# sacs-epfl/decentralizepy

Hardware: AMD Instinct MI355X
Metric: GiB/s fp32 params encoded+decoded (device-resident), 1% top-k (higher is better)
Workload: dtype f32

## Files before the change

### decentralizepy_amd/csrc/dpz_topk.h

```cpp
#pragma once
#include <cstdlib>

#include "dpz_common.h"
#include "dpz_replace.h"

namespace dpz {

struct KeySrc {
  const float* x;
  const float* x0;
  float* acc;
  int mode;
  int rekey;
};

struct Raw4 {
  float4 a, b, q;
  int cnt;
};

template <bool VEC, bool ACC = true>
__device__ __forceinline__ void load_raw4(const KeySrc& s, int64_t i0, int64_t n, Raw4& r) {
  const int64_t rem = n - i0;
  r.cnt = rem >= 4 ? 4 : (rem > 0 ? (int)rem : 0);
// ... 163 lines not shown
  int64_t R = (n + W - 1) / W;
  R = (R + 31) & ~int64_t(31);
  W = (n + R - 1) / R;
  int64_t cap = ((R / 4) + 63) & ~int64_t(63);
  if (k > n / 16) {
    const double frac = 1.25 * (double)k / (double)n + 0.05;
    cap = ((int64_t)(frac * (double)R) + 63) & ~int64_t(63);
    if (cap > ((R + 63) & ~int64_t(63))) cap = (R + 63) & ~int64_t(63);
  }
  if (cap < 64) cap = 64;
  if (k <= n / 16 && cap > 1024) cap = 1024;
  g.W = W; g.B = (W + 3) / 4; g.R = R; g.CAP = cap;
  return g;
}

static inline size_t align256(size_t v) { return (v + 255) & ~size_t(255); }

struct WsLayout {
  size_t ctrl, chist, ex_hist, ex_gt, ex_eq, ex_off, ex_eqb;
  size_t f_ghist, f_segcnt, f_blkabove, f_blkoff, f_cidx, f_ckey, f_cval, f_blcnt, f_blkey, f_blidx;
  size_t total;
  int64_t ex_nblk;
  FastGeom fg;
};

static inline WsLayout ws_layout(int64_t n, int64_t k = 0, int geom = GEOM_LONE) {
  WsLayout L;
  size_t o = 0;
  L.ex_nblk = (n + EX_CHUNK - 1) / EX_CHUNK;
  if (L.ex_nblk < 1) L.ex_nblk = 1;
  L.fg = fast_geom(n > 0 ? n : 1, k, geom);
  L.ctrl = o; o += align256(sizeof(TopkCtrl));
  L.chist = o; o += align256(CB * 4);
  L.ex_hist = o; o += align256(4096 * 4);
  L.ex_gt = o; o += align256(L.ex_nblk * 4);
  L.ex_eq = o; o += align256(L.ex_nblk * 4);
  L.ex_off = o; o += align256(L.ex_nblk * 4);
  L.ex_eqb = o; o += align256(L.ex_nblk * 4);
  L.f_ghist = o; o += align256(GH_COPIES * GH_STRIDE * 4);
  L.f_blcnt = o; o += align256(NSUB * 4);
  L.f_segcnt = o; o += align256(L.fg.W * 4);
  L.f_blkabove = o; o += align256(L.fg.B * 4);
  L.f_blkoff = o; o += align256(L.fg.B * 4);
  L.f_cidx = o; o += align256((size_t)L.fg.W * L.fg.CAP * 4);
  L.f_ckey = o; o += align256((size_t)L.fg.W * L.fg.CAP * 4);
  L.f_cval = o; o += align256((size_t)L.fg.W * L.fg.CAP * 4);
  L.f_blkey = o; o += align256((size_t)BCAP * 4);
  L.f_blidx = o; o += align256((size_t)BCAP * 4);
  L.total = o;
  return L;
}

static inline size_t ws_bytes_needed(int64_t n, int64_t k) {
  size_t m = 0;
  for (int geom = GEOM_LONE; geom <= GEOM_PIPE; ++geom) {
    const size_t t = ws_layout(n, k, geom).total;
    if (t > m) m = t;
// ... 67 lines not shown
```

### decentralizepy_amd/csrc/dpz_topk_sampled.hip

```cpp
#include <cstdio>
#include <cstdlib>

#include "dpz_topk.h"

namespace dpz {

#ifndef DPZ_FILTER_NT
#define DPZ_FILTER_NT 1
#endif

#ifdef DPZ_STAMPS
__device__ unsigned long long g_stamps[64];
#define STAMP_MIN(i) do { if (threadIdx.x == 0) atomicMin(&g_stamps[i], __builtin_amdgcn_s_memrealtime()); } while (0)
#define STAMP_MAX(i) do { __syncthreads(); if (threadIdx.x == 0) atomicMax(&g_stamps[i], __builtin_amdgcn_s_memrealtime()); } while (0)
#define STAMP_ONE(i) do { if (threadIdx.x == 0) g_stamps[i] = __builtin_amdgcn_s_memrealtime(); } while (0)
__device__ unsigned long long g_bst[16][4096];
#define STAMP_T0(i) do { if (threadIdx.x == 0 && blockIdx.x < 4096) g_bst[i][blockIdx.x] = __builtin_amdgcn_s_memrealtime(); } while (0)
__device__ unsigned long long g_fst[6][8192];
#define STAMP_W(i) do { const int64_t _sg = (int64_t)blockIdx.x * 4 + (threadIdx.x >> 6); if ((threadIdx.x & 63) == 0 && _sg < 8192) g_fst[i][_sg] = __builtin_amdgcn_s_memrealtime(); } while (0)
#else
#define STAMP_T0(i) do {} while (0)
#define STAMP_W(i) do {} while (0)
#define STAMP_MIN(i) do {} while (0)
#define STAMP_MAX(i) do {} while (0)
// ... 516 lines not shown
  const int src = m ? (int)__ffsll((long long)m) - 1 : 0;
  *bstar = __shfl(fb, src, 64);
  *need = __shfl(fn, src, 64);
  return ok;
}

template <int NT>
struct SelectLds {
  uint32_t gh[GH_STRIDE];
  uint32_t lkey[SEL_LCAP], lidx[SEL_LCAP];
  uint32_t fbabove[NT / 64 * 2 / 4];
  uint32_t lcnt, gbase, sb_bstar, sb_need, sb_ok;
};

template <bool VEC, int NT = 1024>
__device__ __forceinline__ void sampled_select_kernel_body(SelectLds<NT>& M, KeySrc s, int64_t n, int64_t k, int64_t W, int64_t B, int64_t R, int64_t CAP, TopkCtrl* ctrl, const uint32_t* __restrict__ ghist, const uint32_t* __restrict__ segcnt, const uint32_t* __restrict__ cidx, const uint32_t* __restrict__ ckey, uint32_t* blkabove, uint32_t* blcnt, uint32_t* blkey, uint32_t* blidx, ReplaceJob pj, const uint32_t BID) {
  static_assert(NT == 1024 || NT == 256, "select block: 1024 or 256 threads");
  constexpr int SS = NT / 64 * 2;
  constexpr int NQ = HB / NT;
  {
    const int64_t own = ((W + SEL_SEGS - 1) / SEL_SEGS) * (SEL_SEGS / SS);
    if ((int64_t)BID >= own) {
      replace_block(pj, (int64_t)BID - own);
      return;
    }
  }
  STAMP_MIN(6);
  STAMP_T0(8);
  uint32_t* const gh = M.gh;
  uint32_t* const fbabove = M.fbabove;
  uint32_t* const lkey = M.lkey;
// ... 131 lines not shown
      const int64_t beg = seg * R;
      const int64_t end = (beg + R < n) ? beg + R : n;
      for (int64_t i0 = beg + lane * 4; i0 - lane * 4 < end; i0 += 256) {
        uint32_t key[4];
        const int c = i0 < end ? load_keys4<VEC>(s, i0, end, false, key) : 0;
#pragma unroll
        for (int e = 0; e < 4; ++e) {
          const bool valid = e < c && key[e] >= lo;
          const uint32_t b = valid ? fine_bin(key[e], lo, hi, shift) : 0u;
          above += (uint32_t)__popcll(__ballot(valid && b > bstar));
          append(valid && b == bstar, key[e], (uint32_t)(i0 + e));
        }
      }
    }
    if (lane == 0 && above) atomicAdd(&fbabove[(wid * 2 + u) >> 2], above);
  }
  __syncthreads();
  if (t < SS / 4) {
    const int64_t fb = (int64_t)BID * (SS / 4) + t;
    blkabove[fb] = fb < B ? fbabove[t] : 0u;
  }
  STAMP_T0(10);
  const uint32_t nl = lcnt;
  if (nl) {
    const int sub = (int)(BID & (NSUB - 1));
    if (t == 0) gbase = atomicAdd(&blcnt[sub], nl > SEL_LCAP ? (uint32_t)BCAP : nl);
    __syncthreads();
    const uint32_t gb = gbase;
    for (uint32_t j = t; j < nl && j < SEL_LCAP; j += NT) {
      const uint32_t p = gb + j;
      if (p < SUBCAP) {
        blkey[sub * SUBCAP + p] = lkey[j];
        blidx[sub * SUBCAP + p] = lidx[j];
      }
    }
  }
  STAMP_T0(11);
}

template <bool VEC>
__global__ void __launch_bounds__(1024) sampled_select_kernel(KeySrc s, int64_t n, int64_t k, int64_t W, int64_t B, int64_t R, int64_t CAP, TopkCtrl* ctrl, const uint32_t* __restrict__ ghist, const uint32_t* __restrict__ segcnt, const uint32_t* __restrict__ cidx, const uint32_t* __restrict__ ckey, uint32_t* blkabove, uint32_t* blcnt, uint32_t* blkey, uint32_t* blidx, ReplaceJob pj) {
  __shared__ __attribute__((aligned(16))) SelectLds<1024> lds;
  sampled_select_kernel_body<VEC>(lds, s, n, k, W, B, R, CAP, ctrl, ghist, segcnt, cidx, ckey, blkabove, blcnt, blkey, blidx, pj, (uint32_t)blockIdx.x);
}

__device__ __forceinline__ uint32_t bound_slot(const uint32_t* subbase, uint32_t j) {
  int sb = 0;
#pragma unroll
  for (int u = 1; u < NSUB; ++u) sb += subbase[u] <= j ? 1 : 0;
  return (uint32_t)sb * SUBCAP + (j - subbase[sb]);
}

constexpr int BLDS = 1024;
struct Bound {
  const uint32_t* key;
  const uint32_t* idx;
  const uint32_t* subbase;
  uint32_t* sk;
// ... 146 lines not shown
}

__device__ __forceinline__ uint64_t block_sum64(uint64_t v, uint64_t* wsum64) {
  const int wid = threadIdx.x >> 6, lane = threadIdx.x & 63;
#pragma unroll
  for (int d = 32; d >= 1; d >>= 1) v += __shfl_xor(v, d, 64);
  if (lane == 0) wsum64[wid] = v;
  __syncthreads();
  uint64_t tot = 0;
  for (int w = 0; w < (int)(blockDim.x >> 6); ++w) tot += wsum64[w];
  __syncthreads();
  return tot;
}

template <bool VEC>
__device__ __forceinline__ uint32_t dense_count(const KeySrc s, int64_t seg, int64_t R,
                                                          int64_t n, uint32_t lo, uint32_t T,
                                                          uint32_t icut) {
  const int lane = threadIdx.x & 63;
  const int64_t beg = seg * R;
  const int64_t end = (beg + R < n) ? beg + R : n;
  uint32_t mine = 0;
  for (int64_t i0 = beg + lane * 4; i0 - lane * 4 < end; i0 += 256) {
    uint32_t key[4];
    const int c = i0 < end ? load_keys4<VEC>(s, i0, end, false, key) : 0;
#pragma unroll
    for (int e = 0; e < 4; ++e) {
      const bool f = e < c && key[e] >= lo &&
                     (key[e] > T || (key[e] == T && (uint32_t)(i0 + e) <= icut));
      mine += (uint32_t)__popcll(__ballot(f));
    }
  }
  return mine;
}

template <bool VEC>
__device__ __forceinline__ void dense_write(const KeySrc s, int64_t seg, int64_t R,
                                                      int64_t n, int64_t k, uint32_t lo,
                                                      uint32_t T, uint32_t icut, uint32_t run,
                                                      const float* vals_src, int32_t* idx_out,
                                                      float* val_out, int32_t* counter,
                                                      float* rewind, int val_h,
                                                      uint32_t* slrow) {
  const int lane = threadIdx.x & 63;
  const int64_t beg = seg * R;
  const int64_t end = (beg + R < n) ? beg + R : n;
  for (int64_t i0 = beg + lane * 4; i0 - lane * 4 < end; i0 += 256) {
    uint32_t key[4];
    const int c = i0 < end ? load_keys4<VEC>(s, i0, end, false, key) : 0;
    bool f[4];
    uint32_t pre = 0, tot = 0;
#pragma unroll
// ... 9 lines not shown
    for (int e = 0; e < 4; ++e) {
      if (f[e]) {
        if (pos < (uint64_t)k) {
          const int64_t i = i0 + e;
          idx_out[pos] = (int32_t)i;
          store_val(val_out, val_h, pos, vals_src[i]);
          if (slrow) atomicOr(&slrow[(i - beg) >> 5], 1u << (i & 31));
          if (counter) atomicAdd(&counter[i], 1);
          if (rewind) rewind[i] = 0.0f;
        }
        ++pos;
      }
    }
    run += tot;
  }
}

template <int SPW>
struct CompactCfg {
  static constexpr int CSEG = 4 * SPW;
  static constexpr int PFC = SPW >= 8 ? 1 : 4;
};

#ifndef DPZ_SL_PF
#define DPZ_SL_PF 4
#endif
constexpr int SL_PF = DPZ_SL_PF;
static_assert(32 % SL_PF == 0, "the planes are read in whole steps");

template <int SPW, bool SL>
struct CompactLds {
  uint32_t slrows[SL ? 4 : 1][SL ? (int)(SL_RMAX / 32) : 1];
  uint32_t wcnt[CompactCfg<SPW>::CSEG];
  uint32_t subbase[NSUB + 1];
  uint32_t flag, spec;
  uint64_t wsum64[4];
  alignas(16) ResolveLds RL;
  alignas(16) uint32_t bsk[BLDS];
  alignas(16) uint32_t bsi[BLDS];
};

template <bool VEC, bool PLAIN, int SPW, bool SL>
__device__ __forceinline__ void sampled_compact_kernel_body(CompactLds<SPW, SL>& M, KeySrc s, int64_t n, int64_t k, int64_t W, int64_t R, int64_t CAP, TopkCtrl* ctrl, uint32_t* chist, const uint32_t* __restrict__ blkabove, const uint32_t* __restrict__ blcnt, const uint32_t* __restrict__ blkey, const uint32_t* __restrict__ blidx, const uint32_t* __restrict__ segcnt, const uint32_t* __restrict__ cidx, const uint32_t* __restrict__ ckey, const float* __restrict__ cval, const float* vals_src, int32_t* idx_out, float* val_out, int32_t* counter, float* rewind, int32_t* status_out, ReplaceJob pj, int64_t nrep_first, int val_h, uint32_t* selmask, uint32_t* planes, int64_t nwords, uint32_t* ghist, uint32_t sig, const uint32_t BID) {
  constexpr int CSEG = CompactCfg<SPW>::CSEG;
  constexpr int PFC = CompactCfg<SPW>::PFC;
  uint32_t* const wcnt = M.wcnt;
  uint32_t* const subbase = M.subbase;
  uint32_t& flag = M.flag;
  uint32_t& spec = M.spec;
  uint64_t* const wsum64 = M.wsum64;
  ResolveLds& RL = M.RL;
  uint32_t* const bsk = M.bsk;
  uint32_t* const bsi = M.bsi;
  const int64_t CB_ = (W + CSEG - 1) / CSEG;
  const int64_t B = (W + 3) / 4;
  if (nrep_first > 0 ? (int64_t)BID < nrep_first : (int64_t)BID >= CB_) {
    replace_block(pj, nrep_first > 0 ? (int64_t)BID : (int64_t)BID - CB_);
    return;
// ... 17 lines not shown
  {
    const uint32_t fb0 = (uint32_t)t * 8u;
    uint4 v0 = make_uint4(0, 0, 0, 0), v1 = make_uint4(0, 0, 0, 0);
    if ((int64_t)fb0 < B) {
      v0 = reinterpret_cast<const uint4*>(blkabove)[2 * t];
      v1 = reinterpret_cast<const uint4*>(blkabove)[2 * t + 1];
    }
    const uint32_t v[8] = {v0.x, v0.y, v0.z, v0.w, v1.x, v1.y, v1.z, v1.w};
    const uint32_t fbx = blk * (uint32_t)(CSEG / 4);
#pragma unroll
    for (int q = 0; q < 8; ++q) {
      abv_all += v[q];
      abv_before += fb0 + q < fbx ? v[q] : 0u;
    }
  }
  uint32_t cnt[SPW], kk[SPW][PFC], ii[SPW][PFC];
  float vv[SPW][PFC];
#pragma unroll
  for (int u = 0; u < SPW; ++u) {
    const int64_t seg = seg0 + u;
    cnt[u] = seg < W ? segcnt[seg] : 0u;
#pragma unroll
    for (int c = 0; c < PFC; ++c) {
      kk[u][c] = 0u;
      ii[u][c] = 0u;
      vv[u][c] = 0.f;
    }
    kk[u][0] = seg < W ? ckey[seg * CAP + lane] : 0u;
    ii[u][0] = seg < W ? cidx[seg * CAP + lane] : 0u;
    if (cval && seg < W) vv[u][0] = cval[seg * CAP + lane];
// ... 15 lines not shown
    for (int c = 0; c < PFC; ++c) cc[u][c] = 0u;
#pragma unroll
  for (int u = 0; u < SPW; ++u) {
    const int64_t seg = seg0 + u;
    if (seg < W && cnt[u] != DENSE && (uint32_t)lane < cnt[u]) {
      if (!cval) vv[u][0] = vals_src[ii[u][0]];
      if (PLAIN && counter) cc[u][0] = (uint32_t)counter[ii[u][0]];
    }
  }
  if (t < 64) {
    uint32_t tot;
    const uint32_t ex = wave_excl_scan(sc, &tot);
    const bool over = __ballot(sc > (uint32_t)SUBCAP) != 0;
    const bool spec_ok = __ballot(sc > SPEC) == 0;
    if (t < NSUB) subbase[t] = ex;
    if (t == 0) {
      subbase[NSUB] = tot;
      flag = (over || tot > (uint32_t)BCAP || need_l == 0 || need_l > tot) ? 1u : 0u;
      spec = spec_ok ? 1u : 0u;
    }
  }
  __syncthreads();
  if (flag) {
    if (blk == 0 && t == 0) {
      ctrl->status = 1;
      atomicOr(&ctrl->sticky, 1u);
      if (status_out) *status_out = 1;
    }
    return;
  }
// ... 8 lines not shown
  if (spec) {
    if (sp_slot < subbase[sp_sub + 1] - subbase[sp_sub]) {
      bsk[subbase[sp_sub] + sp_slot] = spk;
      bsi[subbase[sp_sub] + sp_slot] = spi;
    }
    __syncthreads();
  } else {
    bd.load();
  }
  uint32_t T, icut;
  block_resolve(bd, need, lo + (bstar << shift), shift, RL, &T, &icut);
  T = __builtin_amdgcn_readfirstlane(T);
  icut = __builtin_amdgcn_readfirstlane(icut);
  STAMP_T0(2);
  const uint32_t bstart = (uint32_t)((int64_t)blk * CSEG * R);
  uint32_t sb_before = 0, sb_all = 0;
  bd.each([&](uint32_t kv, uint32_t iv) {
    const bool sel = kv > T || (kv == T && iv <= icut);
    sb_all += sel ? 1u : 0u;
    sb_before += (sel && iv < bstart) ? 1u : 0u;
  });
  const uint64_t tot2 = block_sum64(((uint64_t)(abv_all + sb_all) << 32) |
                                        (uint64_t)(abv_before + sb_before), wsum64);
  const uint32_t boff = __builtin_amdgcn_readfirstlane((uint32_t)tot2);
  const uint32_t grand = __builtin_amdgcn_readfirstlane((uint32_t)(tot2 >> 32));
  if (blk == 0 && t == 0) {
    ctrl->T = T;
    ctrl->icut = icut;
    if (grand != (uint32_t)k) {
      ctrl->status = 2;
      atomicOr(&ctrl->sticky, 2u);
    } else if (T > 0u && T < 0x7F800000u) {
      ctrl->hint_T = T;
      ctrl->hint_sig = sig;
    } else {
// ... 14 lines not shown
            kk[u][c] = ckey[seg * CAP + j];
            ii[u][c] = cidx[seg * CAP + j];
            if (cval) vv[u][c] = cval[seg * CAP + j];
          }
        }
#pragma unroll
        for (int c = 1; c < PFC; ++c) {
          const uint32_t j = c * 64u + lane;
          if (j < cnt[u] && !cval) vv[u][c] = vals_src[ii[u][c]];
          if (PLAIN && counter && j < cnt[u]) cc[u][c] = (uint32_t)counter[ii[u][c]];
        }
      }
    }
  }
  auto is_sel = [&](uint32_t key, uint32_t idx) { return key > T || (key == T && idx <= icut); };
#pragma unroll
  for (int u = 0; u < SPW; ++u) {
    const int64_t seg = seg0 + u;
    uint32_t mine = 0;
    if (seg < W && cnt[u] != DENSE) {
#pragma unroll
      for (int c = 0; c < PFC; ++c) {
        const uint32_t j = c * 64u + lane;
        mine += (uint32_t)__popcll(__ballot(j < cnt[u] && is_sel(kk[u][c], ii[u][c])));
      }
      for (uint32_t j0 = PFC * 64u; j0 < cnt[u]; j0 += 4 * 64u) {
        uint32_t kg[4];
#pragma unroll
        for (int g = 0; g < 4; ++g) {
          const uint32_t j = j0 + g * 64u + lane;
          kg[g] = ckey[seg * CAP + (j < cnt[u] ? j : 0u)];
        }
#pragma unroll
        for (int g = 0; g < 4; ++g) {
          const uint32_t j = j0 + g * 64u + lane;
          bool sel = false;
          if (j < cnt[u]) sel = kg[g] > T || (kg[g] == T && cidx[seg * CAP + j] <= icut);
          mine += (uint32_t)__popcll(__ballot(sel));
        }
      }
    } else if (seg < W) {
      mine = dense_count<VEC>(s, seg, R, n, lo, T, icut);
    }
    if (lane == 0) wcnt[wid * SPW + u] = mine;
  }
  __syncthreads();
  STAMP_T0(3);
  uint32_t run = boff;
  for (int w = 0; w < wid * SPW; ++w) run += wcnt[w];
  run = __builtin_amdgcn_readfirstlane(run);
  uint32_t* const slrow = SL ? M.slrows[wid] : nullptr;
#pragma unroll
  for (int u = 0; u < SPW; ++u) {
    const int64_t seg = seg0 + u;
    if (seg >= W) break;
    const int64_t segbeg = seg * R;
    const int segw = SL ? (int)((((segbeg + R < n) ? segbeg + R : n) - segbeg + 31) >> 5) : 0;
    if (SL) {
      for (int j = lane; j < segw; j += 64) slrow[j] = 0u;
      __builtin_amdgcn_wave_barrier();
    }
// ... 29 lines not shown
          const uint32_t j = j0 + g * 64u + lane;
          const uint32_t jc = seg * CAP + (j < cnt[u] ? j : 0u);
          kg[g] = ckey[jc];
          ig[g] = cidx[jc];
          vg[g] = cval ? cval[jc] : 0.f;
        }
#pragma unroll
        for (int g = 0; g < 4; ++g) {
          const uint32_t j = j0 + g * 64u + lane;
          const bool sel = j < cnt[u] && is_sel(kg[g], ig[g]);
          const uint32_t cw = (PLAIN && counter && sel) ? (uint32_t)counter[ig[g]] : 0u;
          emit(sel, ig[g], vg[g], false, cw);
        }
      }
    } else {
      dense_write<VEC>(s, seg, R, n, k, lo, T, icut, run, vals_src, idx_out, val_out, counter,
                       rewind, val_h, slrow);
      run += wcnt[wid * SPW + u];
    }
    if (SL) {
      __builtin_amdgcn_fence(__ATOMIC_RELEASE, "wavefront");
      __builtin_amdgcn_wave_barrier();
      for (int j = lane; j < segw; j += 64) {
        const uint32_t m = slrow[j];
        const int64_t w = (segbeg >> 5) + j;
        selmask[w] = m;
        uint32_t carry = planes ? m : 0u;
        for (int p = 0; p < 32 && carry != 0u; p += SL_PF) {
          uint32_t o[SL_PF];
#pragma unroll
          for (int q = 0; q < SL_PF; ++q) o[q] = planes[(int64_t)(p + q) * nwords + w];
#pragma unroll
          for (int q = 0; q < SL_PF; ++q) {
            if (carry != 0u) {
              planes[(int64_t)(p + q) * nwords + w] = o[q] ^ carry;
              carry &= o[q];
            }
          }
        }
      }
      __builtin_amdgcn_wave_barrier();
    }
  }
  STAMP_T0(4);
}

template <bool VEC, bool PLAIN, int SPW, bool SL>
__global__ void __launch_bounds__(256, SPW >= 8 ? 1 : 4) sampled_compact_kernel(KeySrc s, int64_t n, int64_t k, int64_t W, int64_t R, int64_t CAP, TopkCtrl* ctrl, uint32_t* chist, const uint32_t* __restrict__ blkabove, const uint32_t* __restrict__ blcnt, const uint32_t* __restrict__ blkey, const uint32_t* __restrict__ blidx, const uint32_t* __restrict__ segcnt, const uint32_t* __restrict__ cidx, const uint32_t* __restrict__ ckey, const float* __restrict__ cval, const float* vals_src, int32_t* idx_out, float* val_out, int32_t* counter, float* rewind, int32_t* status_out, ReplaceJob pj, int64_t nrep_first, int val_h, uint32_t* selmask, uint32_t* planes, int64_t nwords, uint32_t* ghist, uint32_t sig) {
  __shared__ __attribute__((aligned(16))) CompactLds<SPW, SL> lds;
  sampled_compact_kernel_body<VEC, PLAIN, SPW, SL>(lds, s, n, k, W, R, CAP, ctrl, chist, blkabove, blcnt, blkey, blidx, segcnt, cidx, ckey, cval, vals_src, idx_out, val_out, counter, rewind, status_out, pj, nrep_first, val_h, selmask, planes, nwords, ghist, sig, (uint32_t)blockIdx.x);
}

static void cosched_shares(double f[3]) {
  f[0] = 0.45; f[1] = 0.55; f[2] = 0.0;
  if (const char* e = DPZ_KNOB_STR(COSCHED)) {
    double v[3];
    if (sscanf(e, "%lf,%lf,%lf", &v[0], &v[1], &v[2]) == 3 && v[0] >= 0 && v[1] >= 0 &&
        v[2] >= 0) {
      const double t = v[0] + v[1] + v[2];
      if (t > 0)
        for (int i = 0; i < 3; ++i) f[i] = v[i] / t;
    }
  }
}

template <bool VEC>
static int run_sampled_t(const EncodeArgs& a, const WsLayout& L, int phases) {
  KeySrc s{a.x, a.x0, a.acc, a.acc_mode, 0};
  TopkCtrl* ctrl = reinterpret_cast<TopkCtrl*>(a.ws + L.ctrl);
  uint32_t* chist = reinterpret_cast<uint32_t*>(a.ws + L.chist);
  uint32_t* ghist = reinterpret_cast<uint32_t*>(a.ws + L.f_ghist);
  uint32_t* segcnt = reinterpret_cast<uint32_t*>(a.ws + L.f_segcnt);
  uint32_t* blkabove = reinterpret_cast<uint32_t*>(a.ws + L.f_blkabove);
  uint32_t* cidx = reinterpret_cast<uint32_t*>(a.ws + L.f_cidx);
  uint32_t* ckey = reinterpret_cast<uint32_t*>(a.ws + L.f_ckey);
  float* cval = (a.vals_src == a.x) ? reinterpret_cast<float*>(a.ws + L.f_cval) : nullptr;
  uint32_t* blcnt = reinterpret_cast<uint32_t*>(a.ws + L.f_blcnt);
  uint32_t* blkey = reinterpret_cast<uint32_t*>(a.ws + L.f_blkey);
  uint32_t* blidx = reinterpret_cast<uint32_t*>(a.ws + L.f_blidx);
  const FastGeom& g = L.fg;
  const unsigned nb = (unsigned)g.B;
  const unsigned nsel = (unsigned)((g.W + SEL_SEGS - 1) / SEL_SEGS);
  ReplaceJob jb[3] = {};
  unsigned pb[3] = {0, 0, 0};
  const int smp_threads = DPZ_KNOB_INT(SAMPLE_THREADS, 256) == 1024 ? 1024 : 256;
  const int smp_blocks = SMP_NCHUNK / (4 * (smp_threads / 64));
  float* copy_out = (a.job && phases == 3 && a.job->scatter) ? a.job->out : nullptr;
  if (a.job && phases == 3) {
// ... 70 lines not shown
#undef DPZ_PIPE2
#undef DPZ_PIPE1
#undef DPZ_PIPE
    } else if (a.acc_mode == DPZ_ACC_NONE)
      DPZ_TIMED(DPZ_KT_TOPK_FILTER, a.st, sampled_filter_kernel<VEC, false, FG><<<nb, 256, 0, a.st>>>(
          s, a.n, r_lo, r_hi, g.W, g.R, g.CAP, ctrl, chist, ghist, segcnt, cidx, ckey, cval,
          copy_out));
    else
      DPZ_TIMED(DPZ_KT_TOPK_FILTER, a.st, sampled_filter_kernel<VEC, true, 3><<<nb, 256, 0, a.st>>>(
          s, a.n, r_lo, r_hi, g.W, g.R, g.CAP, ctrl, chist, ghist, segcnt, cidx, ckey, cval,
          copy_out));
  }
  if (!(phases & 2)) return DPZ_OK;
  s.rekey = 1;
  DPZ_TIMED(DPZ_KT_TOPK_SELECT, a.st, sampled_select_kernel<VEC><<<nsel + pb[1], 1024, 0, a.st>>>(
      s, a.n, a.k, g.W, g.B, g.R, g.CAP, ctrl, ghist, segcnt, cidx, ckey, blkabove, blcnt, blkey,
      blidx, jb[1]));
  float* rewind = (a.acc && a.acc_mode != DPZ_ACC_NONE && !a.selmask) ? a.acc : nullptr;
  const int ablate = (int)DPZ_KNOB_INT(COMPACT_ABLATE, 0);
  if (ablate & 1) rewind = nullptr;
  int32_t* const counter = ((ablate & 2) || a.selmask) ? nullptr : a.counter;
  const bool plain = DPZ_KNOB_INT(COUNTER_PLAIN, a.k > a.n / 32 ? 1 : 0) != 0;
  const int64_t nrep_first = DPZ_KNOB_INT(SCATTER_FIRST, 0) != 0 ? (int64_t)pb[2] : 0;
  const int spw = (int)DPZ_KNOB_INT(COMPACT_SPW, 2);
#define DPZ_COMPACT(PL_, SPW_, SL_)                                                               \
  DPZ_TIMED(DPZ_KT_TOPK_COMPACT, a.st,                                                            \
            (sampled_compact_kernel<VEC, PL_, SPW_, SL_><<<(unsigned)((g.W + 4 * SPW_ - 1) /       \
                                                                     (4 * SPW_)) + pb[2],         \
                                                           256, 0, a.st>>>(                       \
                s, a.n, a.k, g.W, g.R, g.CAP, ctrl, chist, blkabove, blcnt, blkey, blidx, segcnt, \
                cidx, ckey, cval, a.vals_src, a.idx_out, a.val_out, counter, rewind,              \
                a.status_out, jb[2], nrep_first, a.val_h, a.selmask, a.planes, mask_words(a.n),  \
                ghist, sig)))
  if (a.selmask && g.R <= SL_RMAX) {
    DPZ_COMPACT(false, 2, true);
  } else if (plain) {
    if (spw == 8) DPZ_COMPACT(true, 8, false);
    else DPZ_COMPACT(true, 2, false);
  } else {
    if (spw == 8) DPZ_COMPACT(false, 8, false);
    else DPZ_COMPACT(false, 2, false);
  }
#undef DPZ_COMPACT
  return DPZ_OK;
}

// ... 17 lines not shown
}
#endif

struct EncNode {
  const float* x;
  const float* x0;
  int32_t* counter;
  int32_t* idx_out;
  float* val_out;
  char* ws;
  int32_t* status_out;
  uint64_t pad;
};
static_assert(sizeof(EncNode) == 64, "node table entry: 8 x 64-bit words (dpz_codec.h)");
struct WsOff {
  uint64_t ctrl, chist, ghist, segcnt, blkabove, cidx, ckey, cval, blcnt, blkey, blidx;
};

template <class T>
__host__ __device__ __forceinline__ T* wsp(char* ws, uint64_t off) {
  return reinterpret_cast<T*>(ws + off);
}

__global__ void __launch_bounds__(1024) nodes_sample_kernel(const EncNode* __restrict__ tab,
                                                            WsOff o, int64_t n, int nsb) {
  const uint32_t node = blockIdx.x / (uint32_t)nsb, bid = blockIdx.x % (uint32_t)nsb;
  const EncNode e = tab[node];
  KeySrc s{e.x, e.x0, nullptr, DPZ_ACC_NONE, 0};
  sampled_sample_kernel_body(s, n, wsp<TopkCtrl>(e.ws, o.ctrl), wsp<uint32_t>(e.ws, o.chist),
                             wsp<uint32_t>(e.ws, o.ghist), wsp<uint32_t>(e.ws, o.blcnt),
                             ReplaceJob{}, nsb, 0, bid);
// ... 16 lines not shown
}

__global__ void __launch_bounds__(1024) nodes_select_kernel(const EncNode* __restrict__ tab,
                                                            WsOff o, int64_t n, int64_t k,
                                                            int64_t W, int64_t B, int64_t R,
                                                            int64_t CAP, uint32_t nsel) {
  const uint32_t node = blockIdx.x / nsel, bid = blockIdx.x % nsel;
  const EncNode e = tab[node];
  KeySrc s{e.x, e.x0, nullptr, DPZ_ACC_NONE, 1};
  __shared__ __attribute__((aligned(16))) SelectLds<1024> lds;
  sampled_select_kernel_body<true>(
      lds, s, n, k, W, B, R, CAP, wsp<TopkCtrl>(e.ws, o.ctrl),
      wsp<const uint32_t>(e.ws, o.ghist),
      wsp<const uint32_t>(e.ws, o.segcnt), wsp<const uint32_t>(e.ws, o.cidx),
      wsp<const uint32_t>(e.ws, o.ckey), wsp<uint32_t>(e.ws, o.blkabove),
      wsp<uint32_t>(e.ws, o.blcnt), wsp<uint32_t>(e.ws, o.blkey), wsp<uint32_t>(e.ws, o.blidx),
      ReplaceJob{}, bid);
}

#ifndef DPZ_NODES_NO_COUNTER
#define DPZ_NODES_NO_COUNTER 0
#endif
template <bool PLAIN, bool SL>
__global__ void __launch_bounds__(256, 4) nodes_compact_kernel(const EncNode* __restrict__ tab,
                                                               WsOff o, int64_t n, int64_t k,
                                                               int64_t W, int64_t R, int64_t CAP,
                                                               uint32_t ncb, int64_t nwords,
                                                               uint32_t sig) {
  const uint32_t node = blockIdx.x / ncb, bid = blockIdx.x % ncb;
  const EncNode e = tab[node];
  KeySrc s{e.x, e.x0, nullptr, DPZ_ACC_NONE, 1};
  int32_t* const counter = SL || DPZ_NODES_NO_COUNTER ? nullptr : e.counter;
  uint32_t* const selmask = SL ? reinterpret_cast<uint32_t*>(e.pad) : nullptr;
  uint32_t* const planes = SL ? reinterpret_cast<uint32_t*>(e.counter) : nullptr;
  __shared__ __attribute__((aligned(16))) CompactLds<2, SL> lds;
  sampled_compact_kernel_body<true, PLAIN, 2, SL>(
      lds, s, n, k, W, R, CAP, wsp<TopkCtrl>(e.ws, o.ctrl), wsp<uint32_t>(e.ws, o.chist),
      wsp<const uint32_t>(e.ws, o.blkabove), wsp<const uint32_t>(e.ws, o.blcnt),
      wsp<const uint32_t>(e.ws, o.blkey), wsp<const uint32_t>(e.ws, o.blidx),
      wsp<const uint32_t>(e.ws, o.segcnt), wsp<const uint32_t>(e.ws, o.cidx),
      wsp<const uint32_t>(e.ws, o.ckey), wsp<const float>(e.ws, o.cval), e.x, e.idx_out,
      e.val_out, counter, nullptr, e.status_out, ReplaceJob{}, 0, 0, selmask, planes, nwords,
      wsp<uint32_t>(e.ws, o.ghist), sig, bid);
}

int topk_encode_nodes(int m, const void* table, int64_t n, int64_t k, size_t ws_bytes, int flags,
                      hipStream_t st) {
  if (m < 1 || !table || n <= 0 || n >= (int64_t(1) << 31) || k < 1 || k > n) return DPZ_ERR_ARG;
  if (flags & ~(DPZ_TOPK_HINT | DPZ_TOPK_SLICED)) return DPZ_ERR_ARG;
  if (!use_sampled(n, k)) return DPZ_ERR_UNSUPPORTED;
  const bool sl = (flags & DPZ_TOPK_SLICED) != 0;
  if (ws_bytes < ws_bytes_needed(n, k)) return DPZ_ERR_WORKSPACE;
  const WsLayout L = ws_layout(n, k, true);
  const FastGeom& g = L.fg;
  const WsOff o{L.ctrl, L.chist, L.f_ghist, L.f_segcnt, L.f_blkabove, L.f_cidx, L.f_ckey,
                L.f_cval, L.f_blcnt, L.f_blkey, L.f_blidx};
  const EncNode* tab = static_cast<const EncNode*>(table);
  const uint32_t sig = hint_signature(n, k, true, DPZ_ACC_NONE, true);
  const uint32_t hsig = (flags & DPZ_TOPK_HINT) ? sig : 0u;
  const int nsb = SMP_NCHUNK / 16;
  const uint32_t nb = (uint32_t)g.B, nsel = (uint32_t)((g.W + SEL_SEGS - 1) / SEL_SEGS);
  const uint32_t ncb = (uint32_t)((g.W + 7) / 8);
  if ((uint64_t)m * nb >= (1ull << 31) || (uint64_t)m * ncb >= (1ull << 31)) return DPZ_ERR_ARG;
  if (sl && (g.R > SL_RMAX || (g.R & 31) != 0)) return DPZ_ERR_UNSUPPORTED;
  if (!hsig)
    DPZ_TIMED(DPZ_KT_TOPK_SAMPLE, st,
              nodes_sample_kernel<<<(unsigned)(m * nsb), 256, 0, st>>>(tab, o, n, nsb));
  uint32_t r_lo, r_hi;
  window_ranks(n, k, &r_lo, &r_hi);
  if (g.W > 4096)
// ... 108 lines not shown
  }
  uint32_t bid = blockIdx.x;
  if constexpr (FILTER) {
    if (nf) {
      if (bid < nf) {
        sampled_filter_pipe_kernel_body<1, 1, 4, 4, true>(
            lds.f, fs, n, r_lo, r_hi, W, R, CAP, f_ctrl, f_chist, f_ghist, f_segcnt, f_cidx,
            f_ckey, f_cval, f_out, FoldBase{}, f_hsig, f_blcnt, 0, bid);
        return;
      }
      bid -= nf;
    }
  }
  if (bid < nc) {
    sampled_compact_kernel_body<true, false, 2, false>(
        lds.c, cs, n, k, W, R, CAP, c_ctrl, c_chist, c_blkabove, c_blcnt, c_blkey, c_blidx,
        c_segcnt, c_cidx, c_ckey, c_cval, cs.x, c_idx_out, c_val_out, c_counter, nullptr, nullptr,
        c_pj, 0, 0, nullptr, nullptr, 0, c_ghist, sig, bid);
    return;
  }
  bid -= nc;
  if (bid < nsel) {
    sampled_select_kernel_body<true, 256>(lds.s, ss, n, k, W, B, R, CAP, s_ctrl, s_ghist,
                                          s_segcnt, s_cidx, s_ckey, s_blkabove, s_blcnt, s_blkey,
                                          s_blidx, ReplaceJob{}, bid);
    return;
  }
  bid -= nsel;
  if constexpr (FILTER) {
    if (nf) return;
    sampled_filter_pipe_kernel_body<1, 1, 4, 4, true>(
        lds.f, fs, n, r_lo, r_hi, W, R, CAP, f_ctrl, f_chist, f_ghist, f_segcnt, f_cidx, f_ckey,
        f_cval, f_out, FoldBase{}, f_hsig, f_blcnt, 0, bid);
  }
}

bool topk_pipe_ok(int64_t n, int64_t k, size_t ws_bytes) {
  if (n <= 0 || n >= (int64_t(1) << 31) || !use_sampled(n, k) || k > n / 32) return false;
  if (ws_bytes < ws_bytes_needed(n, k)) return false;
  const int64_t wcap = DPZ_KNOB_INT(WPIPE, 0) > W_PIPE ? (int64_t)W_MAX : (int64_t)W_PIPE;
  return fast_geom(n, k, GEOM_PIPE).W <= wcap && DPZ_KNOB_INT(FILTER_PIPE, 1) > 0;
}

int topk_pipe_chain(int p, const PipeStep* c, int64_t n, int64_t k, int64_t r_k, int mode,
                    hipStream_t st) {
  if (p < 1 || !c || !topk_pipe_ok(n, k, ws_bytes_needed(n, k)) || r_k < 1 || r_k > n)
    return DPZ_ERR_ARG;
  const WsLayout L = ws_layout(n, k, GEOM_PIPE);
  const FastGeom& g = L.fg;
  const WsOff o{L.ctrl, L.chist, L.f_ghist, L.f_segcnt, L.f_blkabove, L.f_cidx, L.f_ckey,
                L.f_cval, L.f_blcnt, L.f_blkey, L.f_blidx};
  const uint32_t sig = hint_signature(n, k, GEOM_PIPE, DPZ_ACC_NONE, true);
  const int nsb = SMP_NCHUNK / 16;
  const uint32_t nb = (uint32_t)g.B;
  const uint32_t nsel1024 = (uint32_t)((g.W + SEL_SEGS - 1) / SEL_SEGS);
  const uint32_t nsel256 = nsel1024 * 4;
  const uint32_t ncb = (uint32_t)((g.W + 7) / 8);
  const uint32_t nsc = (uint32_t)((scatter_chunks(r_k) + 3) / 4);
  uint32_t r_lo, r_hi;
  window_ranks(n, k, &r_lo, &r_hi);
  const bool full = mode >= 2;
  const bool ffirst = DPZ_KNOB_INT(PIPE_ORDER, 1) != 0;
  auto* kmerged = pipe_step_kernel<true, PIPE_OCC>;
  auto* kdrain = pipe_step_kernel<false, PIPE_OCC>;
#ifdef DPZ_DIAG
// ... 55 lines not shown
                    KeySrc{fp.x, fp.x0, nullptr, DPZ_ACC_NONE, 0}, fp.ctrl, fp.chist, fp.ghist,
                    fp.segcnt, fp.cidx, fp.ckey, fp.cval, fp.blcnt, fp.out, fp.hsig,
                    KeySrc{sp.x, sp.x0, nullptr, DPZ_ACC_NONE, 1}, sp.ctrl, sp.ghist, sp.segcnt,
                    sp.cidx, sp.ckey, sp.blkabove, sp.blcnt, sp.blkey, sp.blidx,
                    KeySrc{cp.x, cp.x0, nullptr, DPZ_ACC_NONE, 1}, cp.ctrl, cp.chist, cp.blkabove,
                    cp.blcnt, cp.blkey, cp.blidx, cp.segcnt, cp.cidx, cp.ckey, cp.cval, cp.ghist,
                    cp.idx_out, cp.val_out, cp.counter, cp.pj, n, k, r_lo, r_hi, g.W, g.B, g.R,
                    g.CAP, nc, ns, ffirst ? nf : 0u, sig, poison));
    if (!full && fs) {
      KeySrc s{fs->x, fs->x0, nullptr, DPZ_ACC_NONE, 1};
      DPZ_TIMED(DPZ_KT_TOPK_SELECT, st,
                sampled_select_kernel<true><<<nsel1024, 1024, 0, st>>>(
                    s, n, k, g.W, g.B, g.R, g.CAP, wsp<TopkCtrl>(fs->ws, o.ctrl),
                    wsp<const uint32_t>(fs->ws, o.ghist), wsp<const uint32_t>(fs->ws, o.segcnt),
                    wsp<const uint32_t>(fs->ws, o.cidx), wsp<const uint32_t>(fs->ws, o.ckey),
                    wsp<uint32_t>(fs->ws, o.blkabove), wsp<uint32_t>(fs->ws, o.blcnt),
                    wsp<uint32_t>(fs->ws, o.blkey), wsp<uint32_t>(fs->ws, o.blidx), ReplaceJob{}));
    }
  }
  return DPZ_OK;
}

bool fused_foldbase_ok(const EncodeArgs& a, bool vec) {
  return vec && a.acc_mode == DPZ_ACC_NONE && a.x0 && aligned16(a.base_out) &&
         DPZ_KNOB_INT(FILTER_PIPE, 1) > 0 && use_sampled(a.n, a.k) && !a.job;
}

int run_sampled(const EncodeArgs& a, const WsLayout& L, bool vec, int phases) {
  return vec ? run_sampled_t<true>(a, L, phases) : run_sampled_t<false>(a, L, phases);
}

// ... 2 lines not shown
```

Measured before the change: 1518.

## Reuse per-segment above counts from select to skip compact's counting pass

The select kernel now stores each segment's count of keys strictly above the boundary bin into a new workspace array. The compact kernel seeds its per-wave counts from this array and adds boundary-bin selections with shared-memory atomics. This removes the separate pass that re-read candidates, or the dense segment data, just to count selected elements before writing. The cost is an extra workspace array, a per-segment global store, and a reliance on the segabove offset lining up with the layout in the pipelined path.

```diff
diff --git a/decentralizepy_amd/csrc/dpz_topk.h b/decentralizepy_amd/csrc/dpz_topk.h
--- a/decentralizepy_amd/csrc/dpz_topk.h
+++ b/decentralizepy_amd/csrc/dpz_topk.h
@@ -201,11 +201,15 @@
   return g;
 }
 
-static inline size_t align256(size_t v) { return (v + 255) & ~size_t(255); }
+__host__ __device__ static inline size_t align256(size_t v) { return (v + 255) & ~size_t(255); }
+__host__ __device__ static inline size_t segabove_words(int64_t B) {
+  return align256((size_t)B * 4) / 4;
+}
 
 struct WsLayout {
   size_t ctrl, chist, ex_hist, ex_gt, ex_eq, ex_off, ex_eqb;
-  size_t f_ghist, f_segcnt, f_blkabove, f_blkoff, f_cidx, f_ckey, f_cval, f_blcnt, f_blkey, f_blidx;
+  size_t f_ghist, f_segcnt, f_blkabove, f_segabove, f_blkoff, f_cidx, f_ckey, f_cval, f_blcnt;
+  size_t f_blkey, f_blidx;
   size_t total;
   int64_t ex_nblk;
   FastGeom fg;
@@ -228,6 +232,7 @@
   L.f_blcnt = o; o += align256(NSUB * 4);
   L.f_segcnt = o; o += align256(L.fg.W * 4);
   L.f_blkabove = o; o += align256(L.fg.B * 4);
+  L.f_segabove = o; o += align256(L.fg.W * 4);
   L.f_blkoff = o; o += align256(L.fg.B * 4);
   L.f_cidx = o; o += align256((size_t)L.fg.W * L.fg.CAP * 4);
   L.f_ckey = o; o += align256((size_t)L.fg.W * L.fg.CAP * 4);
diff --git a/decentralizepy_amd/csrc/dpz_topk_sampled.hip b/decentralizepy_amd/csrc/dpz_topk_sampled.hip
--- a/decentralizepy_amd/csrc/dpz_topk_sampled.hip
+++ b/decentralizepy_amd/csrc/dpz_topk_sampled.hip
@@ -554,7 +554,7 @@
 };
 
 template <bool VEC, int NT = 1024>
-__device__ __forceinline__ void sampled_select_kernel_body(SelectLds<NT>& M, KeySrc s, int64_t n, int64_t k, int64_t W, int64_t B, int64_t R, int64_t CAP, TopkCtrl* ctrl, const uint32_t* __restrict__ ghist, const uint32_t* __restrict__ segcnt, const uint32_t* __restrict__ cidx, const uint32_t* __restrict__ ckey, uint32_t* blkabove, uint32_t* blcnt, uint32_t* blkey, uint32_t* blidx, ReplaceJob pj, const uint32_t BID) {
+__device__ __forceinline__ void sampled_select_kernel_body(SelectLds<NT>& M, KeySrc s, int64_t n, int64_t k, int64_t W, int64_t B, int64_t R, int64_t CAP, TopkCtrl* ctrl, const uint32_t* __restrict__ ghist, const uint32_t* __restrict__ segcnt, const uint32_t* __restrict__ cidx, const uint32_t* __restrict__ ckey, uint32_t* blkabove, uint32_t* segabove, uint32_t* blcnt, uint32_t* blkey, uint32_t* blidx, ReplaceJob pj, const uint32_t BID) {
   static_assert(NT == 1024 || NT == 256, "select block: 1024 or 256 threads");
   constexpr int SS = NT / 64 * 2;
   constexpr int NQ = HB / NT;
@@ -716,6 +716,7 @@
       }
     }
     if (lane == 0 && above) atomicAdd(&fbabove[(wid * 2 + u) >> 2], above);
+    if (lane == 0 && seg < W) segabove[seg] = above;
   }
   __syncthreads();
   if (t < SS / 4) {
@@ -741,9 +742,9 @@
 }
 
 template <bool VEC>
-__global__ void __launch_bounds__(1024) sampled_select_kernel(KeySrc s, int64_t n, int64_t k, int64_t W, int64_t B, int64_t R, int64_t CAP, TopkCtrl* ctrl, const uint32_t* __restrict__ ghist, const uint32_t* __restrict__ segcnt, const uint32_t* __restrict__ cidx, const uint32_t* __restrict__ ckey, uint32_t* blkabove, uint32_t* blcnt, uint32_t* blkey, uint32_t* blidx, ReplaceJob pj) {
+__global__ void __launch_bounds__(1024) sampled_select_kernel(KeySrc s, int64_t n, int64_t k, int64_t W, int64_t B, int64_t R, int64_t CAP, TopkCtrl* ctrl, const uint32_t* __restrict__ ghist, const uint32_t* __restrict__ segcnt, const uint32_t* __restrict__ cidx, const uint32_t* __restrict__ ckey, uint32_t* blkabove, uint32_t* segabove, uint32_t* blcnt, uint32_t* blkey, uint32_t* blidx, ReplaceJob pj) {
   __shared__ __attribute__((aligned(16))) SelectLds<1024> lds;
-  sampled_select_kernel_body<VEC>(lds, s, n, k, W, B, R, CAP, ctrl, ghist, segcnt, cidx, ckey, blkabove, blcnt, blkey, blidx, pj, (uint32_t)blockIdx.x);
+  sampled_select_kernel_body<VEC>(lds, s, n, k, W, B, R, CAP, ctrl, ghist, segcnt, cidx, ckey, blkabove, segabove, blcnt, blkey, blidx, pj, (uint32_t)blockIdx.x);
 }
 
 __device__ __forceinline__ uint32_t bound_slot(const uint32_t* subbase, uint32_t j) {
@@ -920,28 +921,7 @@
 }
 
 template <bool VEC>
-__device__ __forceinline__ uint32_t dense_count(const KeySrc s, int64_t seg, int64_t R,
-                                                          int64_t n, uint32_t lo, uint32_t T,
-                                                          uint32_t icut) {
-  const int lane = threadIdx.x & 63;
-  const int64_t beg = seg * R;
-  const int64_t end = (beg + R < n) ? beg + R : n;
-  uint32_t mine = 0;
-  for (int64_t i0 = beg + lane * 4; i0 - lane * 4 < end; i0 += 256) {
-    uint32_t key[4];
-    const int c = i0 < end ? load_keys4<VEC>(s, i0, end, false, key) : 0;
-#pragma unroll
-    for (int e = 0; e < 4; ++e) {
-      const bool f = e < c && key[e] >= lo &&
-                     (key[e] > T || (key[e] == T && (uint32_t)(i0 + e) <= icut));
-      mine += (uint32_t)__popcll(__ballot(f));
-    }
-  }
-  return mine;
-}
-
-template <bool VEC>
-__device__ __forceinline__ void dense_write(const KeySrc s, int64_t seg, int64_t R,
+__device__ __forceinline__ uint32_t dense_write(const KeySrc s, int64_t seg, int64_t R,
                                                       int64_t n, int64_t k, uint32_t lo,
                                                       uint32_t T, uint32_t icut, uint32_t run,
                                                       const float* vals_src, int32_t* idx_out,
@@ -981,6 +961,7 @@
     }
     run += tot;
   }
+  return run;
 }
 
 template <int SPW>
@@ -1008,7 +989,7 @@
 };
 
 template <bool VEC, bool PLAIN, int SPW, bool SL>
-__device__ __forceinline__ void sampled_compact_kernel_body(CompactLds<SPW, SL>& M, KeySrc s, int64_t n, int64_t k, int64_t W, int64_t R, int64_t CAP, TopkCtrl* ctrl, uint32_t* chist, const uint32_t* __restrict__ blkabove, const uint32_t* __restrict__ blcnt, const uint32_t* __restrict__ blkey, const uint32_t* __restrict__ blidx, const uint32_t* __restrict__ segcnt, const uint32_t* __restrict__ cidx, const uint32_t* __restrict__ ckey, const float* __restrict__ cval, const float* vals_src, int32_t* idx_out, float* val_out, int32_t* counter, float* rewind, int32_t* status_out, ReplaceJob pj, int64_t nrep_first, int val_h, uint32_t* selmask, uint32_t* planes, int64_t nwords, uint32_t* ghist, uint32_t sig, const uint32_t BID) {
+__device__ __forceinline__ void sampled_compact_kernel_body(CompactLds<SPW, SL>& M, KeySrc s, int64_t n, int64_t k, int64_t W, int64_t R, int64_t CAP, TopkCtrl* ctrl, uint32_t* chist, const uint32_t* __restrict__ blkabove, const uint32_t* __restrict__ segabove, const uint32_t* __restrict__ blcnt, const uint32_t* __restrict__ blkey, const uint32_t* __restrict__ blidx, const uint32_t* __restrict__ segcnt, const uint32_t* __restrict__ cidx, const uint32_t* __restrict__ ckey, const float* __restrict__ cval, const float* vals_src, int32_t* idx_out, float* val_out, int32_t* counter, float* rewind, int32_t* status_out, ReplaceJob pj, int64_t nrep_first, int val_h, uint32_t* selmask, uint32_t* planes, int64_t nwords, uint32_t* ghist, uint32_t sig, const uint32_t BID) {
   constexpr int CSEG = CompactCfg<SPW>::CSEG;
   constexpr int PFC = CompactCfg<SPW>::PFC;
   uint32_t* const wcnt = M.wcnt;
@@ -1056,6 +1037,10 @@
       abv_before += fb0 + q < fbx ? v[q] : 0u;
     }
   }
+  static_assert((CSEG & (CSEG - 1)) == 0, "segment t % CSEG of the block");
+  const uint32_t sgi = blk * (uint32_t)CSEG + ((uint32_t)t & (uint32_t)(CSEG - 1));
+  const uint32_t sab_l = segabove[sgi < (uint32_t)W ? sgi : (uint32_t)W - 1u];
+  const uint32_t sab = sgi < (uint32_t)W ? sab_l : 0u;
   uint32_t cnt[SPW], kk[SPW][PFC], ii[SPW][PFC];
   float vv[SPW][PFC];
 #pragma unroll
@@ -1101,6 +1086,7 @@
     const bool over = __ballot(sc > (uint32_t)SUBCAP) != 0;
     const bool spec_ok = __ballot(sc > SPEC) == 0;
     if (t < NSUB) subbase[t] = ex;
+    if (t < CSEG) wcnt[t] = sab;
     if (t == 0) {
       subbase[NSUB] = tot;
       flag = (over || tot > (uint32_t)BCAP || need_l == 0 || need_l > tot) ? 1u : 0u;
@@ -1139,11 +1125,16 @@
   icut = __builtin_amdgcn_readfirstlane(icut);
   STAMP_T0(2);
   const uint32_t bstart = (uint32_t)((int64_t)blk * CSEG * R);
+  static_assert(CSEG <= 64, "wave 0 stores the block's segment counts");
+  const uint32_t wspan = (uint32_t)(SPW * R);
   uint32_t sb_before = 0, sb_all = 0;
   bd.each([&](uint32_t kv, uint32_t iv) {
     const bool sel = kv > T || (kv == T && iv <= icut);
     sb_all += sel ? 1u : 0u;
     sb_before += (sel && iv < bstart) ? 1u : 0u;
+    const uint32_t d = iv - bstart;
+    if (sel && d < 3u * wspan)
+      atomicAdd(&wcnt[((d >= wspan ? 1u : 0u) + (d >= 2u * wspan ? 1u : 0u)) * SPW], 1u);
   });
   const uint64_t tot2 = block_sum64(((uint64_t)(abv_all + sb_all) << 32) |
                                         (uint64_t)(abv_before + sb_before), wsum64);
@@ -1188,37 +1179,6 @@
     }
   }
   auto is_sel = [&](uint32_t key, uint32_t idx) { return key > T || (key == T && idx <= icut); };
-#pragma unroll
-  for (int u = 0; u < SPW; ++u) {
-    const int64_t seg = seg0 + u;
-    uint32_t mine = 0;
-    if (seg < W && cnt[u] != DENSE) {
-#pragma unroll
-      for (int c = 0; c < PFC; ++c) {
-        const uint32_t j = c * 64u + lane;
-        mine += (uint32_t)__popcll(__ballot(j < cnt[u] && is_sel(kk[u][c], ii[u][c])));
-      }
-      for (uint32_t j0 = PFC * 64u; j0 < cnt[u]; j0 += 4 * 64u) {
-        uint32_t kg[4];
-#pragma unroll
-        for (int g = 0; g < 4; ++g) {
-          const uint32_t j = j0 + g * 64u + lane;
-          kg[g] = ckey[seg * CAP + (j < cnt[u] ? j : 0u)];
-        }
-#pragma unroll
-        for (int g = 0; g < 4; ++g) {
-          const uint32_t j = j0 + g * 64u + lane;
-          bool sel = false;
-          if (j < cnt[u]) sel = kg[g] > T || (kg[g] == T && cidx[seg * CAP + j] <= icut);
-          mine += (uint32_t)__popcll(__ballot(sel));
-        }
-      }
-    } else if (seg < W) {
-      mine = dense_count<VEC>(s, seg, R, n, lo, T, icut);
-    }
-    if (lane == 0) wcnt[wid * SPW + u] = mine;
-  }
-  __syncthreads();
   STAMP_T0(3);
   uint32_t run = boff;
   for (int w = 0; w < wid * SPW; ++w) run += wcnt[w];
@@ -1278,9 +1238,8 @@
         }
       }
     } else {
-      dense_write<VEC>(s, seg, R, n, k, lo, T, icut, run, vals_src, idx_out, val_out, counter,
-                       rewind, val_h, slrow);
-      run += wcnt[wid * SPW + u];
+      run = dense_write<VEC>(s, seg, R, n, k, lo, T, icut, run, vals_src, idx_out, val_out,
+                             counter, rewind, val_h, slrow);
     }
     if (SL) {
       __builtin_amdgcn_fence(__ATOMIC_RELEASE, "wavefront");
@@ -1310,9 +1269,9 @@
 }
 
 template <bool VEC, bool PLAIN, int SPW, bool SL>
-__global__ void __launch_bounds__(256, SPW >= 8 ? 1 : 4) sampled_compact_kernel(KeySrc s, int64_t n, int64_t k, int64_t W, int64_t R, int64_t CAP, TopkCtrl* ctrl, uint32_t* chist, const uint32_t* __restrict__ blkabove, const uint32_t* __restrict__ blcnt, const uint32_t* __restrict__ blkey, const uint32_t* __restrict__ blidx, const uint32_t* __restrict__ segcnt, const uint32_t* __restrict__ cidx, const uint32_t* __restrict__ ckey, const float* __restrict__ cval, const float* vals_src, int32_t* idx_out, float* val_out, int32_t* counter, float* rewind, int32_t* status_out, ReplaceJob pj, int64_t nrep_first, int val_h, uint32_t* selmask, uint32_t* planes, int64_t nwords, uint32_t* ghist, uint32_t sig) {
+__global__ void __launch_bounds__(256, SPW >= 8 ? 1 : 4) sampled_compact_kernel(KeySrc s, int64_t n, int64_t k, int64_t W, int64_t R, int64_t CAP, TopkCtrl* ctrl, uint32_t* chist, const uint32_t* __restrict__ blkabove, const uint32_t* __restrict__ segabove, const uint32_t* __restrict__ blcnt, const uint32_t* __restrict__ blkey, const uint32_t* __restrict__ blidx, const uint32_t* __restrict__ segcnt, const uint32_t* __restrict__ cidx, const uint32_t* __restrict__ ckey, const float* __restrict__ cval, const float* vals_src, int32_t* idx_out, float* val_out, int32_t* counter, float* rewind, int32_t* status_out, ReplaceJob pj, int64_t nrep_first, int val_h, uint32_t* selmask, uint32_t* planes, int64_t nwords, uint32_t* ghist, uint32_t sig) {
   __shared__ __attribute__((aligned(16))) CompactLds<SPW, SL> lds;
-  sampled_compact_kernel_body<VEC, PLAIN, SPW, SL>(lds, s, n, k, W, R, CAP, ctrl, chist, blkabove, blcnt, blkey, blidx, segcnt, cidx, ckey, cval, vals_src, idx_out, val_out, counter, rewind, status_out, pj, nrep_first, val_h, selmask, planes, nwords, ghist, sig, (uint32_t)blockIdx.x);
+  sampled_compact_kernel_body<VEC, PLAIN, SPW, SL>(lds, s, n, k, W, R, CAP, ctrl, chist, blkabove, segabove, blcnt, blkey, blidx, segcnt, cidx, ckey, cval, vals_src, idx_out, val_out, counter, rewind, status_out, pj, nrep_first, val_h, selmask, planes, nwords, ghist, sig, (uint32_t)blockIdx.x);
 }
 
 static void cosched_shares(double f[3]) {
@@ -1336,6 +1295,7 @@
   uint32_t* ghist = reinterpret_cast<uint32_t*>(a.ws + L.f_ghist);
   uint32_t* segcnt = reinterpret_cast<uint32_t*>(a.ws + L.f_segcnt);
   uint32_t* blkabove = reinterpret_cast<uint32_t*>(a.ws + L.f_blkabove);
+  uint32_t* segabove = reinterpret_cast<uint32_t*>(a.ws + L.f_segabove);
   uint32_t* cidx = reinterpret_cast<uint32_t*>(a.ws + L.f_cidx);
   uint32_t* ckey = reinterpret_cast<uint32_t*>(a.ws + L.f_ckey);
   float* cval = (a.vals_src == a.x) ? reinterpret_cast<float*>(a.ws + L.f_cval) : nullptr;
@@ -1436,8 +1396,8 @@
   if (!(phases & 2)) return DPZ_OK;
   s.rekey = 1;
   DPZ_TIMED(DPZ_KT_TOPK_SELECT, a.st, sampled_select_kernel<VEC><<<nsel + pb[1], 1024, 0, a.st>>>(
-      s, a.n, a.k, g.W, g.B, g.R, g.CAP, ctrl, ghist, segcnt, cidx, ckey, blkabove, blcnt, blkey,
-      blidx, jb[1]));
+      s, a.n, a.k, g.W, g.B, g.R, g.CAP, ctrl, ghist, segcnt, cidx, ckey, blkabove, segabove, blcnt,
+      blkey, blidx, jb[1]));
   float* rewind = (a.acc && a.acc_mode != DPZ_ACC_NONE && !a.selmask) ? a.acc : nullptr;
   const int ablate = (int)DPZ_KNOB_INT(COMPACT_ABLATE, 0);
   if (ablate & 1) rewind = nullptr;
@@ -1450,8 +1410,9 @@
             (sampled_compact_kernel<VEC, PL_, SPW_, SL_><<<(unsigned)((g.W + 4 * SPW_ - 1) /       \
                                                                      (4 * SPW_)) + pb[2],         \
                                                            256, 0, a.st>>>(                       \
-                s, a.n, a.k, g.W, g.R, g.CAP, ctrl, chist, blkabove, blcnt, blkey, blidx, segcnt, \
-                cidx, ckey, cval, a.vals_src, a.idx_out, a.val_out, counter, rewind,              \
+                s, a.n, a.k, g.W, g.R, g.CAP, ctrl, chist, blkabove, segabove, blcnt, blkey,      \
+                blidx, segcnt, cidx, ckey, cval, a.vals_src, a.idx_out, a.val_out, counter,       \
+                rewind,                                                                           \
                 a.status_out, jb[2], nrep_first, a.val_h, a.selmask, a.planes, mask_words(a.n),  \
                 ghist, sig)))
   if (a.selmask && g.R <= SL_RMAX) {
@@ -1499,7 +1460,7 @@
 };
 static_assert(sizeof(EncNode) == 64, "node table entry: 8 x 64-bit words (dpz_codec.h)");
 struct WsOff {
-  uint64_t ctrl, chist, ghist, segcnt, blkabove, cidx, ckey, cval, blcnt, blkey, blidx;
+  uint64_t ctrl, chist, ghist, segcnt, blkabove, segabove, cidx, ckey, cval, blcnt, blkey, blidx;
 };
 
 template <class T>
@@ -1546,7 +1507,8 @@
       wsp<const uint32_t>(e.ws, o.ghist),
       wsp<const uint32_t>(e.ws, o.segcnt), wsp<const uint32_t>(e.ws, o.cidx),
       wsp<const uint32_t>(e.ws, o.ckey), wsp<uint32_t>(e.ws, o.blkabove),
-      wsp<uint32_t>(e.ws, o.blcnt), wsp<uint32_t>(e.ws, o.blkey), wsp<uint32_t>(e.ws, o.blidx),
+      wsp<uint32_t>(e.ws, o.segabove), wsp<uint32_t>(e.ws, o.blcnt),
+      wsp<uint32_t>(e.ws, o.blkey), wsp<uint32_t>(e.ws, o.blidx),
       ReplaceJob{}, bid);
 }
 
@@ -1568,7 +1530,8 @@
   __shared__ __attribute__((aligned(16))) CompactLds<2, SL> lds;
   sampled_compact_kernel_body<true, PLAIN, 2, SL>(
       lds, s, n, k, W, R, CAP, wsp<TopkCtrl>(e.ws, o.ctrl), wsp<uint32_t>(e.ws, o.chist),
-      wsp<const uint32_t>(e.ws, o.blkabove), wsp<const uint32_t>(e.ws, o.blcnt),
+      wsp<const uint32_t>(e.ws, o.blkabove), wsp<const uint32_t>(e.ws, o.segabove),
+      wsp<const uint32_t>(e.ws, o.blcnt),
       wsp<const uint32_t>(e.ws, o.blkey), wsp<const uint32_t>(e.ws, o.blidx),
       wsp<const uint32_t>(e.ws, o.segcnt), wsp<const uint32_t>(e.ws, o.cidx),
       wsp<const uint32_t>(e.ws, o.ckey), wsp<const float>(e.ws, o.cval), e.x, e.idx_out,
@@ -1585,7 +1548,8 @@
   if (ws_bytes < ws_bytes_needed(n, k)) return DPZ_ERR_WORKSPACE;
   const WsLayout L = ws_layout(n, k, true);
   const FastGeom& g = L.fg;
-  const WsOff o{L.ctrl, L.chist, L.f_ghist, L.f_segcnt, L.f_blkabove, L.f_cidx, L.f_ckey,
+  const WsOff o{L.ctrl, L.chist, L.f_ghist, L.f_segcnt, L.f_blkabove, L.f_segabove, L.f_cidx,
+                L.f_ckey,
                 L.f_cval, L.f_blcnt, L.f_blkey, L.f_blidx};
   const EncNode* tab = static_cast<const EncNode*>(table);
   const uint32_t sig = hint_signature(n, k, true, DPZ_ACC_NONE, true);
@@ -1724,7 +1688,8 @@
   }
   if (bid < nc) {
     sampled_compact_kernel_body<true, false, 2, false>(
-        lds.c, cs, n, k, W, R, CAP, c_ctrl, c_chist, c_blkabove, c_blcnt, c_blkey, c_blidx,
+        lds.c, cs, n, k, W, R, CAP, c_ctrl, c_chist, c_blkabove,
+        c_blkabove + segabove_words(B), c_blcnt, c_blkey, c_blidx,
         c_segcnt, c_cidx, c_ckey, c_cval, cs.x, c_idx_out, c_val_out, c_counter, nullptr, nullptr,
         c_pj, 0, 0, nullptr, nullptr, 0, c_ghist, sig, bid);
     return;
@@ -1732,7 +1697,8 @@
   bid -= nc;
   if (bid < nsel) {
     sampled_select_kernel_body<true, 256>(lds.s, ss, n, k, W, B, R, CAP, s_ctrl, s_ghist,
-                                          s_segcnt, s_cidx, s_ckey, s_blkabove, s_blcnt, s_blkey,
+                                          s_segcnt, s_cidx, s_ckey, s_blkabove,
+                                          s_blkabove + segabove_words(B), s_blcnt, s_blkey,
                                           s_blidx, ReplaceJob{}, bid);
     return;
   }
@@ -1758,7 +1724,8 @@
     return DPZ_ERR_ARG;
   const WsLayout L = ws_layout(n, k, GEOM_PIPE);
   const FastGeom& g = L.fg;
-  const WsOff o{L.ctrl, L.chist, L.f_ghist, L.f_segcnt, L.f_blkabove, L.f_cidx, L.f_ckey,
+  const WsOff o{L.ctrl, L.chist, L.f_ghist, L.f_segcnt, L.f_blkabove, L.f_segabove, L.f_cidx,
+                L.f_ckey,
                 L.f_cval, L.f_blcnt, L.f_blkey, L.f_blidx};
   const uint32_t sig = hint_signature(n, k, GEOM_PIPE, DPZ_ACC_NONE, true);
   const int nsb = SMP_NCHUNK / 16;
@@ -1844,7 +1811,8 @@
                     s, n, k, g.W, g.B, g.R, g.CAP, wsp<TopkCtrl>(fs->ws, o.ctrl),
                     wsp<const uint32_t>(fs->ws, o.ghist), wsp<const uint32_t>(fs->ws, o.segcnt),
                     wsp<const uint32_t>(fs->ws, o.cidx), wsp<const uint32_t>(fs->ws, o.ckey),
-                    wsp<uint32_t>(fs->ws, o.blkabove), wsp<uint32_t>(fs->ws, o.blcnt),
+                    wsp<uint32_t>(fs->ws, o.blkabove), wsp<uint32_t>(fs->ws, o.segabove),
+                    wsp<uint32_t>(fs->ws, o.blcnt),
                     wsp<uint32_t>(fs->ws, o.blkey), wsp<uint32_t>(fs->ws, o.blidx), ReplaceJob{}));
     }
   }
```

Result: no change. 1516 (median of 2 runs) (-0.1%).
